# modassarrana89/authorino

Measured on AMD Instinct MI355X. Metric: request×rule evals/sec (+ allow/deny decisions/sec, % HBM roofline), higher is better.
Workload: dtype u8

## Files before the change

### authorino_amd/csrc/ajx_lean.h

```cpp
#pragma once
#include "ajx_lean_cls.h"

namespace ajx {
namespace lean {

#if !defined(__HIP_DEVICE_COMPILE__) && defined(AJX_LEAN_COUNT)
inline uint64_t g_lean_iters = 0, g_lean_subs = 0;
inline uint32_t* g_lean_trace = nullptr;
inline uint32_t g_lean_trace_n = 0, g_lean_trace_cap = 0;
#define AJX_LEAN_TICK(x) (x)++
#define AJX_LEAN_TRACE(k) \
    (g_lean_trace && g_lean_trace_n < g_lean_trace_cap ? (void)(g_lean_trace[g_lean_trace_n++] = (uint32_t)(g_lean_subs << 8 | (k))) : (void)0)
#else
#define AJX_LEAN_TICK(x) ((void)0)
#define AJX_LEAN_TRACE(k) ((void)0)
#endif
constexpr uint32_t kRingStride = 128;
constexpr uint32_t kChunkStride = 64 * 16;
constexpr uint32_t kRingBytesPerWave = 64 * kRingStride;
constexpr uint32_t kMaxLive = 16;
constexpr uint32_t kIdxKeyLen = kIndexKeyLen;

enum : uint32_t { S_RUN = 0, S_DONE = 1, S_SLOW = 2 };

template <bool ARR = true, bool CAPS = true>
struct Walk {
    const TrieNode* tn;
    const KeySlot* ks;
    const uint8_t* lits;
    uint32_t ks_mask, ks_probes, ks_mult, ks_shift;
    const uint8_t* a16;
    uint32_t mis;
    const uint8_t* ring;
    RowRef row;
    uint32_t st, depth;
    uint32_t kinds;
    uint64_t nlo, nhi;
    uint32_t top, tarr;
    AJX_HD uint32_t ta() const { return ARR ? tarr : 0u; }
    uint32_t expk;
    uint32_t pend;
    uint32_t idx, asv, nasv;
    uint32_t skipw, skips;
    uint32_t caps, cap0s, cap1s, ncap;
    uint32_t carry_oq;
    uint32_t lbs1;
    uint64_t found;
    const EagerSel* eg;
    uint64_t eT, eD;
    uint32_t keep;

    AJX_HD uint32_t ro(uint32_t a) const { return ((a & 0x70u) << 6) | (a & 15u); }
    AJX_HD uint32_t rw(uint32_t q) const { return *reinterpret_cast<const uint32_t*>(ring + ro(q & 127u)); }
    AJX_HD uint32_t rb(uint32_t p) const { return ring[ro((p + mis) & 127u)]; }
    AJX_HD uint32_t r32(uint32_t a) const {
        const uint32_t q = a & ~3u, sh = a & 3u;
        const uint32_t w0 = rw(q), w1 = rw(q + 4);
#if defined(__HIP_DEVICE_COMPILE__)
        return __builtin_amdgcn_alignbyte(w1, w0, sh);
#else
        return sh ? (w0 >> (8 * sh)) | (w1 << (32 - 8 * sh)) : w0;
#endif
    }
    AJX_HD uint64_t r64(uint32_t a) const {
        const uint32_t q = a & ~3u, sh = a & 3u;
        const uint32_t w0 = rw(q), w1 = rw(q + 4), w2 = rw(q + 8);
#if defined(__HIP_DEVICE_COMPILE__)
        const uint32_t lo = __builtin_amdgcn_alignbyte(w1, w0, sh), hi = __builtin_amdgcn_alignbyte(w2, w1, sh);
#else
        const uint32_t lo = sh ? (w0 >> (8 * sh)) | (w1 << (32 - 8 * sh)) : w0;
        const uint32_t hi = sh ? (w1 >> (8 * sh)) | (w2 << (32 - 8 * sh)) : w1;
#endif
        return (uint64_t)lo | ((uint64_t)hi << 32);
    }
    AJX_HD static bool any_lane(bool x) {
#if defined(__HIP_DEVICE_COMPILE__)
        return __builtin_amdgcn_ballot_w64(x) != 0;
#else
        return x;
#endif
    }
    AJX_HD uint32_t node_at(uint32_t dd) const {
        const uint32_t k = dd - 1;
        const uint64_t w = k < 8 ? nlo : nhi;
        return (uint32_t)(w >> ((k & 7) * 8)) & 0xFFu;
    }
    AJX_HD int32_t leaf_sel(uint32_t node) const {
        if (node == kNoNode) return -1;
        const int32_t s = tn[node].selector;
        if (s < 0 || ((found >> s) & 1)) return -1;
        return s;
    }
    AJX_HD void record(int32_t s, uint32_t start, uint32_t end, uint32_t type, uint32_t esc, uint64_t v0 = 0) {
        found |= 1ull << s;
        bool dec = false;
        const bool lit = type == T_TRUE || type == T_FALSE || type == T_NULL;
        if (eg && ((type == T_STRING && !esc) || lit)) {
            const EagerSel e = eg[s];
            const uint64_t v1 = r64((start + 8u + mis) & 127u);
            const uint64_t b16 = rb(start + 16u);
            const uint64_t c0 = (v0 >> 8) | (v1 << 56), c1 = (v1 >> 8) | (b16 << 56);
            const uint32_t mt = lit ? lit_match(e, type) : eager_match(e, end - start - 2u, c0, c1);
#pragma unroll
            for (int k = 0; k < 2; k++) {
                const uint32_t m = e.m[k], op = (m >> 8) & 0xFFu;
                const uint64_t bit = 1ull << (m & 63u);
                const bool yes = ((mt >> k) & 1u) == (op == OP_EQ || op == OP_INCL ? 1u : 0u);
                eD = (m & kEagerValid) ? eD | bit : eD;
                eT = (m & kEagerValid) && yes ? eT | bit : eT;
            }
            dec = (e.pad[0] & kEagerAll) != 0 && !(keep && (e.pad[0] & kEagerKeep));
        }
        if (!dec)
            row[1 + (uint32_t)s] =
                (uint64_t)start | ((uint64_t)(((end - start) & 0xFFFFFFu) | (type << 24) | (esc << 27)) << 32);
    }
    AJX_HD static uint32_t lit_match(const EagerSel& e, uint32_t type) {
        const uint32_t litb = type == T_TRUE ? (uint32_t)kLitTrue : type == T_FALSE ? (uint32_t)kLitFalse
                                                                                    : (uint32_t)kLitEmpty;
        uint32_t r = 0;
#pragma unroll
        for (int k = 0; k < 2; k++) {
            const uint32_t m = e.m[k], op = (m >> 8) & 0xFFu;
            const bool arr = op == OP_INCL || op == OP_EXCL;
            r |= ((m >> 24) & litb) && !(type == T_NULL && arr) ? 1u << k : 0u;
        }
        return r;
    }
    AJX_HD static uint32_t eager_match(const EagerSel& e, uint32_t cl, uint64_t c0, uint64_t c1) {
        const uint64_t m0 = cl >= 8 ? ~0ull : ((1ull << (8 * cl)) - 1ull);
        const uint64_t m1 = cl >= 16 ? ~0ull : (cl > 8 ? ((1ull << (8 * (cl - 8))) - 1ull) : 0ull);
        uint32_t r = 0;
#pragma unroll
        for (int k = 0; k < 2; k++) {
            const uint64_t l0 = (uint64_t)e.lit[k][0] | ((uint64_t)e.lit[k][1] << 32);
            const uint64_t l1 = (uint64_t)e.lit[k][2] | ((uint64_t)e.lit[k][3] << 32);
            const bool eq = (e.m[k] & kEagerValid) && cl == ((e.m[k] >> 16) & 0xFFu) && ((c0 ^ l0) & m0) == 0 &&
                            ((c1 ^ l1) & m1) == 0;
            r |= eq ? 1u << k : 0u;
        }
        return r;
    }
    AJX_HD uint32_t lookup(uint64_t sig, uint32_t len, uint32_t parent, uint32_t kstart, int32_t ring_lo) const {
        const uint32_t want = len | (parent << 16);
        uint32_t h = (uint32_t)sig ^ (((uint32_t)(sig >> 32) << 13) | ((uint32_t)(sig >> 32) >> 19)) ^ (len << 24) ^
                     (parent << 16);
        h = (h * ks_mult) >> ks_shift;
        const bool longk = len > 8 && len != kIdxKeyLen;
        uint32_t node = kNoNode;
        for (uint32_t t = 0; t < ks_probes; t++) {
            struct alignas(16) SlotHalves {
                uint64_t sig, rest;
            };
            const SlotHalves q = *reinterpret_cast<const SlotHalves*>(&ks[(h + t) & ks_mask]);
            KeySlot sl;
            sl.sig = q.sig;
            sl.meta = (uint32_t)q.rest;
            sl.key_off8 = (uint16_t)(q.rest >> 32);
            sl.facts = (uint16_t)(q.rest >> 48);
            bool hit = (sl.meta != kEmptySlot) & (sl.sig == sig) & ((sl.meta & 0xFFFFFFu) == want);
            if (hit && longk) {
                const uint8_t* kl = lits + (uint32_t)sl.key_off8 * 8u;
                hit = (int32_t)kstart >= ring_lo ? key_head_equal(kstart, len - 8, kl) : key_rest_equal(kstart, len - 8, kl);
            }
            node = hit ? (sl.meta >> 24) | ((uint32_t)sl.facts << 8) : node;
        }
        return node;
    }
    AJX_HD bool key_head_equal(uint32_t k0, uint32_t cnt, const uint8_t* kl) const {
        bool eq = true;
        for (uint32_t k = 0; k < cnt; k += 8) {
            const uint32_t r = cnt - k;
            const uint64_t m = r >= 8 ? ~0ull : ((1ull << (8 * r)) - 1ull);
            const uint64_t b = (uint64_t)load_u32_any(kl + k) | ((uint64_t)load_u32_any(kl + k + 4) << 32);
            eq = eq && ((r64((k0 + k + mis) & 127u) ^ b) & m) == 0;
        }
        return eq;
    }
    AJX_COLD bool key_rest_equal(uint32_t k0, uint32_t cnt, const uint8_t* kl) const {
        for (uint32_t k = 0; k < cnt; k++)
            if (a16[mis + k0 + k] != kl[k]) return false;
        return true;
    }
    AJX_HD void close(uint32_t p) {
        if (CAPS && ncap) {
            const uint32_t cs = ncap == 2 ? caps >> 16 : caps & 0xFFFFu, start = ncap == 2 ? cap1s : cap0s;
            if ((cs >> 8) == depth) {
                row[1 + (cs & 0xFFu)] =
                    (uint64_t)start | ((uint64_t)(((p + 1 - start) & 0xFFFFFFu) | ((uint32_t)T_JSON << 24)) << 32);
                ncap--;
            }
        }
        depth--;
        if (depth == 0) {
            st = S_DONE;
            pend = p;
            return;
        }
        top = node_at(depth);
        tarr = ARR ? (kinds >> depth) & 1u : 0u;
        expk = 1;
        if (ARR && tarr) {
            idx = nasv == 2 ? asv >> 16 : asv & 0xFFFFu;
            nasv--;
        }
    }
    AJX_HD bool has_bs(uint32_t a, uint32_t b, const Sub& c, const Sub& l) const {
        if (lbs1 > a) return true;
        const uint64_t bs = (uint64_t)c.bs | ((uint64_t)l.bs << 32);
        const int32_t ra = (int32_t)a - c.base, rbb = (int32_t)b - c.base;
        uint64_t m = rbb >= 64 ? ~0ull : ((1ull << rbb) - 1ull);
        if (ra > 0) m &= ~((1ull << ra) - 1ull);
        return (bs & m) != 0;
    }

    AJX_HD uint32_t node_facts(uint32_t node) const {
        if (node == kNoNode) return 0u;
        const TrieNode t = tn[node];
        return ((uint32_t)(t.selector + 1) & kSlotSelMask) | (t.n_children ? kSlotKids : 0u) |
               ((t.flags & 1u) ? kSlotArrKids : 0u);
    }
    AJX_HD void open_f(uint32_t node, uint32_t nf, bool arr, uint32_t p) {
        int32_t s = (int32_t)(nf & kSlotSelMask) - 1;
        if (s >= 0 && ((found >> s) & 1)) s = -1;
        if (node == kNoNode || !(nf & kSlotKids) || (arr && !(nf & kSlotArrKids))) {
            skipw = 1u | ((s >= 0 ? (uint32_t)s + 1u : 0u) << 24);
            skips = p;
            return;
        }
        if (depth + 1 > kMaxLive) { st = S_SLOW; return; }
        if (ARR && tarr) {
            if (nasv >= 2 || idx > 0xFFFFu) { st = S_SLOW; return; }
            asv = nasv == 1 ? (asv & 0xFFFFu) | (idx << 16) : nasv == 0 ? (asv & 0xFFFF0000u) | idx : asv;
            nasv++;
        }
        depth++;
        const uint32_t k = depth - 1;
        const uint64_t m = 0xFFull << ((k & 7) * 8), x = (uint64_t)node << ((k & 7) * 8);
        const uint64_t lo = nlo, hi = nhi;
        nlo = k < 8 ? (lo & ~m) | x : lo;
        nhi = k < 8 ? hi : (hi & ~m) | x;
        if (ARR) kinds = arr ? kinds | (1u << depth) : kinds & ~(1u << depth);
        top = node;
        tarr = ARR && arr ? 1u : 0u;
        expk = 1;
        idx = 0;
        if (CAPS && s >= 0) {
            found |= 1ull << s;
            if (ncap >= 2) { st = S_SLOW; return; }
            const uint32_t v = (uint32_t)s | (depth << 8);
            caps = ncap == 1 ? (caps & 0xFFFFu) | (v << 16) : ncap == 0 ? (caps & 0xFFFF0000u) | v : caps;
            cap1s = ncap == 1 ? p : cap1s;
            cap0s = ncap == 0 ? p : cap0s;
            ncap++;
        }
    }

    AJX_HD void walk(const Sub& c, Sub& l) {
        uint32_t T;
        if (skipw) {
            const int32_t rel = (int32_t)skips - c.base;
            const uint32_t ex = rel < 0 ? ~0u : above((uint32_t)rel);
            const uint32_t o = popc(c.op & ex), x = popc(c.cl & ex);
            if (x < (skipw & 0xFFFFFFu)) {
                skipw += o - x;
                T = 0;
            } else {
                uint32_t br = (c.op | c.cl) & ex, dep = skipw & 0xFFFFFFu, b = 0;
                while (dep && br) {
                    b = ctz(br);
                    br &= br - 1u;
                    dep = (c.op >> b) & 1u ? dep + 1u : dep - 1u;
                }
                if (dep) {
                    skipw = (skipw & 0xFF000000u) | dep;
                    T = 0;
                } else {
                    if (skipw >> 24) record((int32_t)(skipw >> 24) - 1, skips, (uint32_t)c.base + b + 1u, T_JSON, 0);
                    skipw = 0;
                    T = c.tok & above(b);
                }
            }
        } else {
            T = c.tok;
        }
        const uint32_t cok = (c.co >> 1) | (l.co << 31);
        const uint32_t cb = (uint32_t)c.base;
        const uint64_t cl64 = (uint64_t)c.cl | ((uint64_t)l.cl << 32);
        constexpr uint32_t kNone = 0xFFFFFFFFu;
#if defined(AJX_LEAN_AB_NO_BSGUARD)
        const bool bsw = true;
#else
        const bool bsw = any_lane((c.bs | l.bs) != 0 || lbs1 > carry_oq);
#endif
        AJX_LEAN_TICK(g_lean_subs);
        while (T) {
            AJX_LEAN_TICK(g_lean_iters);
            const uint32_t i = ctz(T);
            T &= T - 1u;
            const uint32_t p = cb + i;
            uint32_t after = kNone;
            bool bad = false;
            {
                const bool bq = (c.cq >> i) & 1u, bo = (c.op >> i) & 1u, bc = (c.cl >> i) & 1u, kq = (cok >> i) & 1u;
                const bool root = depth == 0;
                const bool key = bq && !ta() && expk;
                const bool pv = bq && !ta() && !expk;
                const bool el = ta() && !bc;
                bad = root ? !(bo && p == 0) : bq ? kq != key : bc ? false : !ta();
                const uint32_t oqb = c.oq & below(i);
                const uint32_t ss = oqb ? cb + hib(oqb) : carry_oq;
                const uint32_t k0 = ss + 1u, klen = p - k0;
                const uint32_t vs = key ? p + 2u : pv ? (pend & 0xFFFFFFu) : bq ? ss : p;
                uint64_t sig = r64((p - 8u + mis) & 127u);
                const uint64_t v0 = r64((vs + mis) & 127u);
                const uint32_t vb = bq && !key ? (uint32_t)'"' : (uint32_t)v0 & 0xFFu;
                if (key && !bad) bad = klen >= kIdxKeyLen || (bsw && has_bs(k0, p, c, l));
                uint32_t lk = kNoNode;
                const bool eidx = ARR && el;
                if ((key && !bad) || eidx) {
                    sig = klen >= 8 ? sig : (klen ? sig >> (8 * (8 - klen)) : 0ull);
                    lk = lookup(key ? sig : (uint64_t)idx, key ? klen : kIdxKeyLen, top, k0, (int32_t)cb - 32);
                }
                idx += el ? 1u : 0u;
                uint32_t node = lk & 0xFFu, nf = lk >> 8;
#if defined(AJX_LEAN_AB_TN_FACTS)
                node = pv ? pend >> 24 : root ? 0u : node;
                nf = node_facts(node);
#else
                if (pv || root) {
                    node = pv ? pend >> 24 : 0u;
                    nf = node_facts(node);
                }
#endif
                int32_t s = (int32_t)(nf & kSlotSelMask) - 1;
                if (s >= 0 && ((found >> s) & 1)) s = -1;
                const bool vstr = bq && (!key || vb == '"');
                const bool vopen = key ? (vb == '{' || vb == '[') : bo;
                const bool vscal = !bq && !bo && !bc ? true : key && !vstr && !vopen;
                if (bc) bad |= root || ta() != (vb == ']' ? 1u : 0u) || (!ta() && !expk);
                uint32_t e = p;
                bool ended = true;
                const uint32_t rv = vs - cb;
                if (key && vstr) {
                    const uint64_t m = ((uint64_t)c.cq | ((uint64_t)l.cq << 32)) & (~0ull << (rv + 1));
                    if (m) {
                        const uint32_t j = (uint32_t)__builtin_ctzll(m);
                        if (j < 32) T &= ~(1u << j);
                        else l.tok &= ~(1u << (j - 32));
                        e = cb + j;
                    } else {
                        ended = false;
                        expk = 0;
                        pend = vs | (node << 24);
                    }
                }
                if (pv) expk = 1;
                if (vstr && ended) after = e + 1u;
                uint32_t type = T_STRING, end = e + 1u;
                if (vscal && !bad) {
                    const bool lit = vb == 't' || vb == 'f' || (vb == 'n' && ((uint32_t)v0 >> 8 & 0xFFu) == 'u');
                    const uint32_t r = vs - cb;
                    const uint64_t stm = (uint64_t)c.st | ((uint64_t)l.st << 32);
                    const uint64_t m = r >= 63 ? 0ull : stm & (~0ull << (r + 1));
                    end = cb + (uint32_t)__builtin_ctzll(m | (1ull << 63));
                    after = m ? end : kNone;
                    if (!scalar_start(vb)) {
                        bad = true;
                    } else if (s >= 0 || (el && lit)) {
                        const uint32_t len = end - vs;
                        type = T_NUMBER;
                        if (lit) {
                            const uint64_t w = v0;
                            const bool ok = vb == 't' ? len == 4 && (uint32_t)w == 0x65757274u
                                          : vb == 'f' ? len == 5 && (w & 0xFFFFFFFFFFull) == 0x65736C6166ull
                                                      : len == 4 && (uint32_t)w == 0x6C6C756Eu;
                            type = vb == 't' ? T_TRUE : vb == 'f' ? T_FALSE : T_NULL;
                            bad |= !ok;
                        }
                        bad |= m == 0;
                    }
                }
                if (!bad && s >= 0 && ((vstr && ended) || vscal))
                    record(s, vs, end, type, vstr && bsw && has_bs(vs, e, c, l) ? 1u : 0u, v0);
                if (!bad && vopen) {
                    if (key) {
                        if (rv < 32) T &= ~(1u << rv);
                        else l.tok &= ~(1u << (rv - 32));
                    }
                    open_f(node, nf, vb == '[', vs);
                    const uint32_t ip = key ? rv : i;
                    T = ip < 32 ? T & above(ip) : 0u;
                    after = vs + 1u;
                    if (skipw) {
                        bad |= root;
                        after = kNone;
                        if (ip < 32) {
                            uint32_t br = (c.op | c.cl) & above(ip), dep = 1;
                            while (br) {
                                const uint32_t b = ctz(br);
                                br &= br - 1u;
                                dep = (c.op >> b) & 1u ? dep + 1u : dep - 1u;
                                if (dep == 0) {
                                    if (skipw >> 24) record((int32_t)(skipw >> 24) - 1, skips, cb + b + 1u, T_JSON, 0);
                                    skipw = 0;
                                    T &= above(b);
                                    after = cb + b + 1u;
                                    break;
                                }
                            }
                            if (skipw) {
                                skipw = (skipw & 0xFF000000u) | dep;
                                T = 0;
                            }
                        }
                    }
                }
                if (!bad && bc) {
                    close(p);
                    after = p + 1u;
                }
                AJX_LEAN_TRACE(bc ? 8 : bo ? (root ? 6 : 7) : pv ? 2 : key ? (vstr ? 3 : vopen ? 4 : 5) : bq ? 1 : 9);
            }
            while (!bad && st == S_RUN && after != kNone) {
                const uint32_t r = after - cb;
                if (r >= 64 || !((cl64 >> r) & 1u)) break;
                bad = depth == 0 || ta() != (rb(after) == ']' ? 1u : 0u) || (!ta() && !expk);
                if (bad) break;
                if (r < 32) T &= ~(1u << r);
                else l.tok &= ~(1u << (r - 32));
                close(after);
                after++;
            }
            if (bad) st = S_SLOW;
            if (st != S_RUN) T = 0;
        }
        if (c.oq) carry_oq = (uint32_t)c.base + hib(c.oq);
        if (c.bs) lbs1 = (uint32_t)c.base + hib(c.bs) + 1u;
    }
};

template <int ABL = 0, bool ARR = true, bool CAPS = true, class Loader>
AJX_HD bool scan_doc(const uint8_t* blob, uint32_t n, uint32_t mis, RowRef row, uint8_t* ring, Loader& ld,
                     uint64_t dec[2], uint32_t keep = 1) {
    const RulesetHdr* h = (const RulesetHdr*)blob;
    Walk<ARR, CAPS> w;
    w.tn = reinterpret_cast<const TrieNode*>(blob + uni(h->off_trie_nodes));
    w.ks = reinterpret_cast<const KeySlot*>(blob + uni(h->off_key_slots));
    w.lits = blob + uni(h->off_literals);
    w.ks_mask = uni((1u << h->key_slots_log2) - 1u);
    w.ks_probes = uni(h->key_probes);
    w.ks_mult = uni(h->key_mult);
    w.ks_shift = uni(32u - h->key_slots_log2);
    w.a16 = ld.base();
    w.mis = mis;
    w.ring = ring;
    w.row = row;
    w.st = S_RUN;
    w.depth = 0;
    w.kinds = 0;
    w.nlo = w.nhi = ~0ull;
    w.top = kNoNode;
    w.tarr = 0;
    w.expk = 1;
    w.pend = (uint32_t)kNoNode << 24;
    w.idx = w.asv = w.nasv = 0;
    w.skipw = w.skips = 0;
    w.caps = w.cap0s = w.cap1s = w.ncap = 0;
    w.carry_oq = 0;
    w.lbs1 = 0;
    w.found = 0;
    w.eg = ABL != 3 && uni(h->off_eager) ? reinterpret_cast<const EagerSel*>(blob + uni(h->off_eager)) : nullptr;
    w.eT = w.eD = 0;
    w.keep = keep;
    Carry cr;
    cr.f = 0;
    cr.bad = 0x7FFFFFFF;

    const uint32_t nblk = (n + mis + 15) / 16;
    const uint32_t nwin = (nblk + 3) / 4;
    auto valid_of = [&](int32_t base) -> uint32_t {
        uint32_t v = ~0u;
        if (base < 0) v &= ~below((uint32_t)(-base));
        const int32_t hi = (int32_t)n - base;
        if (hi < 32) v &= hi <= 0 ? 0u : below((uint32_t)hi);
        return v;
    };
    auto issue_half = [&](uint32_t win, uint32_t k) {
        const uint32_t c = (win & 1u) * 4u + 2u * k;
        ld.issue(win * 4u + 2u * k, c);
        ld.issue(win * 4u + 2u * k + 1u, c + 1u);
    };
    auto half_words = [&](uint32_t c, uint32_t x[8]) {
        const Block16 a = *reinterpret_cast<const Block16*>(ring + c * kChunkStride);
        const Block16 b = *reinterpret_cast<const Block16*>(ring + (c + 1u) * kChunkStride);
        x[0] = a.x, x[1] = a.y, x[2] = a.z, x[3] = a.w, x[4] = b.x, x[5] = b.y, x[6] = b.z, x[7] = b.w;
    };
    Sub s0, s1, s2;
    uint32_t ck = 0;
    issue_half(0, 0);
    issue_half(0, 1);
    ld.template wait<0>();
    {
        uint32_t x[8];
        half_words(0, x);
        if constexpr (ABL == 1) ck ^= x[0] ^ x[5];
        else classify(s0, x, -(int32_t)mis, valid_of(-(int32_t)mis), cr);
        half_words(2, x);
        if constexpr (ABL == 1) ck ^= x[2] ^ x[7];
        else classify(s1, x, 32 - (int32_t)mis, valid_of(32 - (int32_t)mis), cr);
    }
    for (uint32_t win = 0; win < nwin; win++) {
        const int32_t b0 = (int32_t)(win * 64u) - (int32_t)mis;
        const bool more = win + 1 < nwin;
        const uint32_t c2 = ((win + 1) & 1u) * 4u;
        if (more) issue_half(win + 1, 0);
        if constexpr (ABL != 1 && ABL != 2) {
            w.walk(s0, s1);
            if (w.st != S_RUN) break;
        }
        if (more) issue_half(win + 1, 1);
        if (more) {
            ld.template wait<2>();
            uint32_t x[8];
            half_words(c2, x);
            if constexpr (ABL == 1) ck ^= x[1] ^ x[6];
            else classify(s2, x, b0 + 64, valid_of(b0 + 64), cr);
        } else {
            s2.base = b0 + 64;
            s2.tok = s2.cq = s2.oq = s2.op = s2.cl = s2.co = s2.st = s2.bs = 0;
        }
        if constexpr (ABL != 1 && ABL != 2) {
            w.walk(s1, s2);
            if (w.st != S_RUN) break;
        } else if constexpr (ABL == 2) {
            ck ^= s0.tok ^ s0.bs ^ s1.tok ^ s1.bs;
        }
        if (more) {
            ld.template wait<0>();
            uint32_t x[8];
            half_words(c2 + 2u, x);
            if constexpr (ABL == 1) ck ^= x[3] ^ x[4];
            else classify(s1, x, b0 + 96, valid_of(b0 + 96), cr);
        }
        s0 = s2;
    }
    if constexpr (ABL == 1 || ABL == 2) {
        row[0] = (uint64_t)ck ^ ((uint64_t)(uint32_t)cr.bad << 32) ^ s0.tok ^ s1.tok;
        dec[0] = dec[1] = 0;
        return true;
    }
    ld.template wait<0>();
    if (w.st != S_DONE || cr.bad <= (int32_t)w.pend) {
        row[0] = kRowSlow;
        return false;
    }
    row[0] = w.found;
    dec[0] = w.eD;
    dec[1] = w.eT;
    return true;
}

#if defined(__HIPCC__)
struct DmaLoader {
    const uint4* a4;
    uint32_t nblk;
    uint8_t* wave_ring;
    __device__ const uint8_t* base() const { return reinterpret_cast<const uint8_t*>(a4); }
    __device__ void issue(uint32_t b, uint32_t chunk) const {
        __builtin_amdgcn_global_load_lds(
                (const void*)(a4 + (b < nblk ? b : nblk - 1u)),
                (__attribute__((address_space(3))) void*)(wave_ring + chunk * kChunkStride), 16, 0, 0);
    }
    template <int K>
    __device__ void wait() const {
        if constexpr (K == 0) asm volatile("s_waitcnt vmcnt(0)" ::: "memory");
        else asm volatile("s_waitcnt vmcnt(2)" ::: "memory");
    }
};
#endif
struct CopyLoader {
    const uint8_t* a16;
    uint32_t nblk, avail;
    uint8_t* lane_ring;
    AJX_HD const uint8_t* base() const { return a16; }
    AJX_HD void issue(uint32_t b, uint32_t chunk) const {
        const uint32_t bb = b < nblk ? b : nblk - 1u;
        uint8_t* dst = lane_ring + chunk * kChunkStride;
        for (uint32_t i = 0; i < 16; i++) dst[i] = bb < avail ? a16[16 * bb + i] : 0;
    }
    template <int K>
    AJX_HD void wait() const {}
};

}
}
```

Before: 14.30 billion.

## Let idle lanes borrow tokens from the lookahead sub-chunk while the wave is busy

The token walk now tracks a 64-bit token mask spanning the current and next 32-byte sub-chunk. On device, lanes that have finished their own tokens keep processing tokens from the next sub-chunk while any lane in the wave still has work, provided an early_ok check says the token can be handled without context. The aim is to reduce divergence idle time in the lockstep wavefront loop. It also adds host-side tracing and spare-budget instrumentation, a check for a closing quote followed by a colon, and it adds complexity and risk of state errors at the chunk boundary.

```diff
diff --git a/authorino_amd/csrc/ajx_lean.h b/authorino_amd/csrc/ajx_lean.h
--- a/authorino_amd/csrc/ajx_lean.h
+++ b/authorino_amd/csrc/ajx_lean.h
@@ -8,12 +8,34 @@
 inline uint64_t g_lean_iters = 0, g_lean_subs = 0;
 inline uint32_t* g_lean_trace = nullptr;
 inline uint32_t g_lean_trace_n = 0, g_lean_trace_cap = 0;
+inline uint32_t* g_lean_trace_pos = nullptr;
+constexpr uint32_t kTraceElig = 1u << 24, kTraceStop = 1u << 25, kTraceEarly = 1u << 26;
+constexpr uint32_t kTraceSplit = 1u << 27;
+#if !defined(AJX_LEAN_SPARE_DEFAULT)
+#define AJX_LEAN_SPARE_DEFAULT 0
+#endif
+inline uint32_t g_lean_spare_policy = AJX_LEAN_SPARE_DEFAULT, g_lean_spare_k = 0;
+inline uint64_t g_lean_spare_rng = 1, g_lean_early = 0;
+inline uint32_t lean_spare_draw() {
+    if (g_lean_spare_policy == 1) return g_lean_spare_k;
+    if (g_lean_spare_policy == 2) return ~0u;
+    if (g_lean_spare_policy != 3) return 0;
+    uint64_t x = g_lean_spare_rng;
+    x ^= x << 13, x ^= x >> 7, x ^= x << 17;
+    g_lean_spare_rng = x;
+    return (uint32_t)((x >> 33) % 5u);
+}
 #define AJX_LEAN_TICK(x) (x)++
-#define AJX_LEAN_TRACE(k) \
-    (g_lean_trace && g_lean_trace_n < g_lean_trace_cap ? (void)(g_lean_trace[g_lean_trace_n++] = (uint32_t)(g_lean_subs << 8 | (k))) : (void)0)
+#define AJX_LEAN_TRACE(k, pos) \
+    (g_lean_trace && g_lean_trace_n < g_lean_trace_cap \
+         ? (void)((g_lean_trace_pos ? (void)(g_lean_trace_pos[g_lean_trace_n] = (pos)) : (void)0), \
+                  g_lean_trace[g_lean_trace_n++] = (uint32_t)(g_lean_subs << 8 | (k))) \
+         : (void)0)
+#define AJX_LEAN_SPARE() lean_spare_draw()
 #else
 #define AJX_LEAN_TICK(x) ((void)0)
-#define AJX_LEAN_TRACE(k) ((void)0)
+#define AJX_LEAN_TRACE(k, pos) ((void)0)
+#define AJX_LEAN_SPARE() 0u
 #endif
 constexpr uint32_t kRingStride = 128;
 constexpr uint32_t kChunkStride = 64 * 16;
@@ -256,6 +278,15 @@
         }
     }
 
+    AJX_HD static bool early_ok(const Sub& l, uint32_t j) {
+        if (j >= 31) return false;
+        const uint32_t v = j + 2u;
+        if ((l.cq >> j) & (l.co >> (j + 1u)) & 1u)
+            return v < 32 && ((((l.oq | l.op) >> v) & 1u) || (l.st & above(v)) != 0);
+        if (!(((l.cq | l.op | l.cl) >> j) & 1u)) return (l.st & above(j)) != 0;
+        return true;
+    }
+
     AJX_HD void walk(const Sub& c, Sub& l) {
         uint32_t T;
         if (skipw) {
@@ -284,9 +315,10 @@
         } else {
             T = c.tok;
         }
-        const uint32_t cok = (c.co >> 1) | (l.co << 31);
         const uint32_t cb = (uint32_t)c.base;
-        const uint64_t cl64 = (uint64_t)c.cl | ((uint64_t)l.cl << 32);
+        const uint64_t cq64 = (uint64_t)c.cq | ((uint64_t)l.cq << 32), op64 = (uint64_t)c.op | ((uint64_t)l.op << 32);
+        const uint64_t cl64 = (uint64_t)c.cl | ((uint64_t)l.cl << 32), oq64 = (uint64_t)c.oq | ((uint64_t)l.oq << 32);
+        const uint64_t co64 = (uint64_t)c.co | ((uint64_t)l.co << 32);
         constexpr uint32_t kNone = 0xFFFFFFFFu;
 #if defined(AJX_LEAN_AB_NO_BSGUARD)
         const bool bsw = true;
@@ -294,22 +326,46 @@
         const bool bsw = any_lane((c.bs | l.bs) != 0 || lbs1 > carry_oq);
 #endif
         AJX_LEAN_TICK(g_lean_subs);
-        while (T) {
+        uint64_t T64 = (uint64_t)T | ((uint64_t)l.tok << 32);
+#if defined(AJX_LEAN_AB_NO_BORROW)
+        bool go = false;
+#else
+        bool go = !skipw;
+#endif
+        uint32_t spare = AJX_LEAN_SPARE();
+        (void)spare;
+        for (;;) {
+            const bool own = (uint32_t)T64 != 0;
+#if defined(AJX_LEAN_AB_NO_BORROW)
+            if (!own) break;
+#elif defined(__HIP_DEVICE_COMPILE__)
+            if (!any_lane(own)) break;
+#else
+            if (!own && !(go && T64 && spare)) break;
+            if (!own) spare--;
+#endif
+            const uint32_t i = (uint32_t)__builtin_ctzll(T64 | (1ull << 63));
+            if (!own) go = go && T64 && early_ok(l, i - 32u);
+            if (!own && !go) continue;
             AJX_LEAN_TICK(g_lean_iters);
-            const uint32_t i = ctz(T);
-            T &= T - 1u;
+#if !defined(__HIP_DEVICE_COMPILE__) && defined(AJX_LEAN_COUNT)
+            g_lean_early += own ? 0u : 1u;
+            const uint32_t tr_el = (i >= 32 ? early_ok(l, i - 32u) : early_ok(c, i)) ? kTraceElig : 0u;
+            uint32_t tr_kind = 0, tr_split = 0;
+#endif
+            T64 &= T64 - 1ull;
             const uint32_t p = cb + i;
             uint32_t after = kNone;
             bool bad = false;
             {
-                const bool bq = (c.cq >> i) & 1u, bo = (c.op >> i) & 1u, bc = (c.cl >> i) & 1u, kq = (cok >> i) & 1u;
+                const bool bq = (cq64 >> i) & 1u, bo = (op64 >> i) & 1u, bc = (cl64 >> i) & 1u, kq = ((co64 >> i) >> 1) & 1u;
                 const bool root = depth == 0;
                 const bool key = bq && !ta() && expk;
                 const bool pv = bq && !ta() && !expk;
                 const bool el = ta() && !bc;
                 bad = root ? !(bo && p == 0) : bq ? kq != key : bc ? false : !ta();
-                const uint32_t oqb = c.oq & below(i);
-                const uint32_t ss = oqb ? cb + hib(oqb) : carry_oq;
+                const uint64_t oqb = oq64 & ((1ull << i) - 1ull);
+                const uint32_t ss = oqb ? cb + 63u - (uint32_t)__builtin_clzll(oqb) : carry_oq;
                 const uint32_t k0 = ss + 1u, klen = p - k0;
                 const uint32_t vs = key ? p + 2u : pv ? (pend & 0xFFFFFFu) : bq ? ss : p;
                 uint64_t sig = r64((p - 8u + mis) & 127u);
@@ -343,12 +399,15 @@
                 bool ended = true;
                 const uint32_t rv = vs - cb;
                 if (key && vstr) {
-                    const uint64_t m = ((uint64_t)c.cq | ((uint64_t)l.cq << 32)) & (~0ull << (rv + 1));
-                    if (m) {
-                        const uint32_t j = (uint32_t)__builtin_ctzll(m);
-                        if (j < 32) T &= ~(1u << j);
-                        else l.tok &= ~(1u << (j - 32));
+                    const uint64_t m = cq64 & ((~0ull << (rv & 63u)) << 1);
+                    const uint32_t j = (uint32_t)__builtin_ctzll(m | (1ull << 63));
+                    if (j < 63) {
+                        T64 &= ~(1ull << j);
                         e = cb + j;
+                        bad |= ((co64 >> j) >> 1) & 1u;
+#if !defined(__HIP_DEVICE_COMPILE__) && defined(AJX_LEAN_COUNT)
+                        if (i < 32 && j >= 32) tr_split = kTraceSplit;
+#endif
                     } else {
                         ended = false;
                         expk = 0;
@@ -384,17 +443,14 @@
                 if (!bad && s >= 0 && ((vstr && ended) || vscal))
                     record(s, vs, end, type, vstr && bsw && has_bs(vs, e, c, l) ? 1u : 0u, v0);
                 if (!bad && vopen) {
-                    if (key) {
-                        if (rv < 32) T &= ~(1u << rv);
-                        else l.tok &= ~(1u << (rv - 32));
-                    }
                     open_f(node, nf, vb == '[', vs);
                     const uint32_t ip = key ? rv : i;
-                    T = ip < 32 ? T & above(ip) : 0u;
+                    T64 = ip < 63 ? T64 & (~0ull << (ip + 1u)) : 0ull;
                     after = vs + 1u;
                     if (skipw) {
                         bad |= root;
                         after = kNone;
+                        go = false;
                         if (ip < 32) {
                             uint32_t br = (c.op | c.cl) & above(ip), dep = 1;
                             while (br) {
@@ -404,37 +460,44 @@
                                 if (dep == 0) {
                                     if (skipw >> 24) record((int32_t)(skipw >> 24) - 1, skips, cb + b + 1u, T_JSON, 0);
                                     skipw = 0;
-                                    T &= above(b);
+                                    T64 &= ~0ull << (b + 1u);
                                     after = cb + b + 1u;
+#if !defined(AJX_LEAN_AB_NO_BORROW)
+                                    go = true;
+#endif
                                     break;
                                 }
                             }
-                            if (skipw) {
-                                skipw = (skipw & 0xFF000000u) | dep;
-                                T = 0;
-                            }
+                            if (skipw) skipw = (skipw & 0xFF000000u) | dep;
                         }
+                        if (skipw) T64 &= ~0xFFFFFFFFull;
                     }
                 }
                 if (!bad && bc) {
                     close(p);
                     after = p + 1u;
                 }
-                AJX_LEAN_TRACE(bc ? 8 : bo ? (root ? 6 : 7) : pv ? 2 : key ? (vstr ? 3 : vopen ? 4 : 5) : bq ? 1 : 9);
+#if !defined(__HIP_DEVICE_COMPILE__) && defined(AJX_LEAN_COUNT)
+                tr_kind = bc ? 8 : bo ? (root ? 6 : 7) : pv ? 2 : key ? (vstr ? 3 : vopen ? 4 : 5) : bq ? 1 : 9;
+#endif
             }
             while (!bad && st == S_RUN && after != kNone) {
                 const uint32_t r = after - cb;
                 if (r >= 64 || !((cl64 >> r) & 1u)) break;
                 bad = depth == 0 || ta() != (rb(after) == ']' ? 1u : 0u) || (!ta() && !expk);
                 if (bad) break;
-                if (r < 32) T &= ~(1u << r);
-                else l.tok &= ~(1u << (r - 32));
+                T64 &= ~(1ull << r);
                 close(after);
                 after++;
             }
             if (bad) st = S_SLOW;
-            if (st != S_RUN) T = 0;
-        }
+            if (st != S_RUN) {
+                T64 &= ~0xFFFFFFFFull;
+                go = false;
+            }
+            AJX_LEAN_TRACE(tr_kind, p | tr_el | tr_split | (go ? 0u : kTraceStop) | (own ? 0u : kTraceEarly));
+        }
+        l.tok = (uint32_t)(T64 >> 32);
         if (c.oq) carry_oq = (uint32_t)c.base + hib(c.oq);
         if (c.bs) lbs1 = (uint32_t)c.base + hib(c.bs) + 1u;
     }
```

After: 15.60 billion, median of 6. 9.1% higher.
